# torgeiba/CPUPerformanceRayTracer

Measured on AMD Instinct MI355X. Metric: ray-samples/sec (pixels×spp×bounces) at 1920×1080; ms/frame, higher is better.
Workload: dtype f32; 1 GPU; c2_1080p; width=1920, height=1080, spp=8, bounces=8, parallelism=single GPU, step=one launch accumulating 8 frames (spp) of every pixel in HBM

## Files before the change

### cpuperformanceraytracer_amd/_native.py

```python
from __future__ import annotations

import ctypes
import os
from pathlib import Path

from .build import LIB as _LIB_PATH

PT_OK = 0
PT_EINVAL = -1
PT_EHIP = -2
PT_ENOMEM = -3
PT_ESTATE = -4
PT_EKERNEL = -5

PT_LAYOUT_INTERLEAVED = 0
PT_LAYOUT_PLANAR8 = 1
PT_LAYOUT_TILED_PLANAR8 = 2

PT_FLAG_DEFER_READBACK = 1
PT_FLAG_PIN_HOST = 2
PT_FLAG_GATHER_ROOT = 4

PT_MAX_DEVICES = 16

PT_PIXEL_RGBA8 = 0
PT_PIXEL_XRGB8 = 1

EXPORTED_SYMBOLS = (
    "pt_init", "pt_shutdown", "pt_last_error", "pt_default_config", "pt_set_frame", "pt_get_frame",
    "pt_render_scalar", "pt_render_simd", "pt_render_simd_tiled", "pt_render_tile", "pt_begin_frame",
    "pt_readback", "pt_gather_root", "pt_unpin_host", "pt_release_buffer", "pt_initialized_device", "pt_check_device_errors", "pt_build_checked", "pt_device_count",
    "pt_device_ordinal", "pt_render_device", "pt_render_device_chain", "pt_chain_counts", "pt_count_device", "pt_render_device_present", "pt_launch_variant",
    "pt_cam_cache_query",
    "pt_load_texture", "pt_decode_hdr", "pt_free_texture", "pt_set_env_map", "pt_render_simt_textured",
    "pt_tonemap", "pt_tonemap_device", "pt_write_bmp", "pt_load_cubemap_texture",
    "pt_v4_default_config", "pt_v4_set_config", "pt_v4_get_config", "pt_v4_initialize_global_render_resources",
    "pt_v4_reinitialize_render_tile_data", "pt_v4_initialize_scene", "pt_v4_clear_scene", "pt_v4_add_material",
    "pt_v4_add_quad", "pt_v4_add_sphere", "pt_v4_set_frame", "pt_v4_get_frame", "pt_v4_get_scene_tables", "pt_render_opt_v4",
    "pt_copy_output_to_file", "pt_v4_render_device", "pt_v4_render_device_chain", "pt_v4_count_device", "pt_v4_begin_frame",
    "pt_make_work_queue", "pt_add_work_queue_entry", "pt_complete_all_work", "pt_complete_all_work_async",
    "pt_wait_work", "pt_work_queue_size", "pt_free_work_queue",
)

PT_RENDERER_SIMD_TILED = 0
PT_RENDERER_SIMT_TEXTURED = 1
PT_RENDERER_V4 = 2

PT_V4_ENV_NONE = 0
PT_V4_ENV_EQUIRECT = 1
PT_V4_ENV_CUBEMAP = 2
PT_V4_MAX_OBJECTS = 12


class PtConfig(ctypes.Structure):
    _fields_ = [("device", ctypes.c_int32), ("num_bounces", ctypes.c_int32),
                ("samples_per_frame", ctypes.c_int32), ("flags", ctypes.c_uint32),
# ... 81 lines not shown
        "pt_set_frame": (i32, [u32]),
        "pt_get_frame": (u32, []),
        "pt_render_scalar": (i32, [vp, i32, i32, i32]),
        "pt_render_simd": (i32, [vp, i32, i32, i32]),
        "pt_render_simd_tiled": (i32, [vp, i32, i32, i32, i32, i32, i32, i32]),
        "pt_render_tile": (i32, [ctypes.POINTER(PtBufferInfo), ctypes.POINTER(PtTileInfo)]),
        "pt_begin_frame": (i32, []),
        "pt_readback": (i32, [vp]),
        "pt_gather_root": (i32, [vp, ctypes.POINTER(vp)]),
        "pt_unpin_host": (i32, [vp]),
        "pt_release_buffer": (i32, [vp]),
        "pt_initialized_device": (i32, []),
        "pt_check_device_errors": (i32, []),
        "pt_build_checked": (i32, []),
        "pt_device_count": (i32, []),
        "pt_device_ordinal": (i32, [i32]),
        "pt_render_device": (i32, [ctypes.POINTER(PtDeviceJob), vp]),
        "pt_count_device": (i32, [ctypes.POINTER(PtDeviceJob), vp, ctypes.POINTER(PtWorkCounts)]),
        "pt_render_device_present": (i32, [ctypes.POINTER(PtDeviceJob), vp, i32, vp]),
        "pt_render_device_chain": (i32, [ctypes.POINTER(PtDeviceJob), vp]),
        "pt_chain_counts": (i32, [ctypes.POINTER(ctypes.c_uint64), ctypes.POINTER(ctypes.c_uint64)]),
        "pt_launch_variant": (i32, [ctypes.POINTER(PtDeviceJob), ctypes.POINTER(i32), ctypes.POINTER(i32)]),
        "pt_cam_cache_query": (i32, [ctypes.POINTER(PtDeviceJob), vp, ctypes.POINTER(i32), ctypes.POINTER(ctypes.c_uint64)]),
        "pt_load_texture": (i32, [ctypes.c_char_p, ctypes.POINTER(PtTexture)]),
        "pt_decode_hdr": (i32, [vp, ctypes.c_size_t, ctypes.POINTER(PtTexture)]),
        "pt_free_texture": (None, [ctypes.POINTER(PtTexture)]),
        "pt_set_env_map": (i32, [ctypes.POINTER(PtTexture)]),
        "pt_render_simt_textured": (i32, [vp, i32, i32, i32, i32, i32, i32, i32, ctypes.POINTER(PtTexture)]),
        "pt_tonemap": (i32, [vp, i32, i32, i32, i32, i32, vp, i32]),
        "pt_tonemap_device": (i32, [vp, i32, i32, i32, i32, i32, vp, i32, vp]),
        "pt_write_bmp": (i32, [ctypes.c_char_p, i32, i32, i32, vp]),
        "pt_load_cubemap_texture": (i32, [ctypes.POINTER(ctypes.c_char_p), ctypes.POINTER(PtTexture)]),
        "pt_v4_default_config": (None, [ctypes.POINTER(PtV4Config)]),
        "pt_v4_set_config": (i32, [ctypes.POINTER(PtV4Config)]),
        "pt_v4_get_config": (i32, [ctypes.POINTER(PtV4Config)]),
        "pt_v4_initialize_global_render_resources": (i32, []),
        "pt_v4_reinitialize_render_tile_data": (i32, []),
        "pt_v4_initialize_scene": (i32, []),
        "pt_v4_clear_scene": (i32, []),
        "pt_v4_add_material": (i32, [ctypes.POINTER(PtV4Material)]),
        "pt_v4_add_quad": (i32, [ctypes.POINTER(ctypes.c_float)]),
        "pt_v4_add_sphere": (i32, [ctypes.POINTER(ctypes.c_float)]),
        "pt_v4_set_frame": (i32, [u32]),
        "pt_v4_get_frame": (u32, []),
        "pt_v4_get_scene_tables": (i32, [vp, i32, ctypes.POINTER(i32), ctypes.POINTER(i32)]),
        "pt_render_opt_v4": (i32, [vp, i32, i32, i32, i32, i32, i32, i32, ctypes.POINTER(PtTexture), vp]),
# ... 31 lines not shown
```

### cpuperformanceraytracer_amd/build.py

```python
from __future__ import annotations

import os
import shutil
import subprocess
import sys
from pathlib import Path

PKG = Path(__file__).resolve().parent
ROOT = PKG.parent
CSRC = PKG / "csrc"
LIB = PKG / "libpt_mi355.so"
ARCH = os.environ.get("PT_OFFLOAD_ARCH", "gfx950")

SOURCES = ["pt_kernel.hip", "pt_output.hip", "pt_v4.hip", "pt_scene.cpp", "pt_v4_scene.cpp", "pt_capi.cpp",
           "pt_dropin.cpp", "pt_texture.cpp"]
HEADERS = ["pt_kernel.h", "pt_output.h", "pt_v4.h", "pt_v4_default_scene.h", "pt_scene.h", "pt_sincosf.h", "pt_exactmath.h",
           "pt_invtrig.h", "pt_envcert.h", "pt_tile_queue.h", "pt_quadcull.h", "pt_libmf.h", "pt_wave.h", "pt_guard.h",
           "pt_chain.h", "pt_camcache.h"]
CHECKED_LIB = ROOT / "build" / "libpt_checked.so"
PARITY_FLAGS = [
    "-ffp-contract=off",
    "-fhip-fp32-correctly-rounded-divide-sqrt",
    "-fno-gpu-flush-denormals-to-zero",
]
PERF_FLAGS = ["-mllvm", "-amdgpu-atomic-optimizer-strategy=None", "-fno-slp-vectorize"]


def hipcc() -> str:
    for cand in (os.environ.get("HIPCC"), "/opt/rocm/bin/hipcc", shutil.which("hipcc")):
        if cand and Path(cand).exists():
            return cand
    raise RuntimeError("hipcc not found (ROCm required to build libpt_mi355.so)")


def _stale(target: Path, deps) -> bool:
    if not target.exists():
        return True
    t = target.stat().st_mtime
    return any(Path(d).stat().st_mtime > t for d in deps)


# ... 89 lines not shown
```

### cpuperformanceraytracer_amd/csrc/pt_capi.cpp

```cpp
#include "pt_kernel.h"
#include "pt_guard.h"
#include "pt_output.h"
#include "pt_v4.h"
#include "../../include/pt_mi355.h"
#include <stdarg.h>
#include <stdio.h>
#include <stdlib.h>
#include <string.h>
#include <new>
#include <vector>

namespace {

struct SchedKey {
    int32_t kind = 0;
    int32_t width = 0, height = 0, col0 = 0, ncols = 0, row_start = 0, row_stride = 0, nrows = 0, bounces = 0;
    const float* env = nullptr;
    uint32_t ntiles = 0;
    uint32_t split = 0;
    bool operator==(const SchedKey& o) const
    {
        return kind == o.kind && width == o.width && height == o.height && col0 == o.col0 && ncols == o.ncols &&
               row_start == o.row_start && row_stride == o.row_stride && nrows == o.nrows && bounces == o.bounces &&
               env == o.env && ntiles == o.ntiles && split == o.split;
    }
};
struct Sched {
    bool used = false;
    hipStream_t stream = nullptr;
    SchedKey key;
    uint32_t* cost = nullptr;
    uint32_t* order = nullptr;
    uint32_t* units = nullptr;
    bool have_cost = false;
    bool built = false;
    unsigned long long launches = 0;
    unsigned long long last_use = 0;
    hipEvent_t tune_ev[2 * 18] = {};
    uint32_t tuned = 0;
    uint32_t narms = 0;
    int32_t tune_nframes = 0;
    int8_t wide = -1;
    uint32_t* epoch = nullptr;
    uint32_t chain_seq = 0;
    unsigned long long* cam = nullptr;
    bool cam_off = false;
    uint8_t cam_state = 0;
};
enum : uint8_t { kCamEmpty = 0, kCamFilled = 1, kCamSettled = 2 };
constexpr uint32_t kTuneRounds = 3;
constexpr int kSchedSlots = 16;
constexpr int kBands = 4;
constexpr uint32_t kSchedMinTiles = 512;
constexpr unsigned kQueueRing = 256;
constexpr unsigned long long kSchedRebuildDefault = 256;

struct Dev {
    int32_t ordinal = 0;
    hipStream_t stream = nullptr;
    PtScene* dscene = nullptr;
    float* dbuf = nullptr;
    size_t dbuf_cap = 0;
    unsigned long long* dcounters = nullptr;
    uint32_t* derr = nullptr;
    float* dct = nullptr;
    uint32_t dct_waves = 0;
    int ct_slot = -1;
    uint32_t* herr = nullptr;
    unsigned int* dqueue = nullptr;
    unsigned queue_next = 0;
    bool queue_pre_zeroed = false;
    hipStream_t last_stream = nullptr;
    hipStream_t queue_stream[kQueueRing] = {};
    hipEvent_t queue_event[kQueueRing] = {};
    int16_t queue_alias[kQueueRing];
    float* denv = nullptr;
    Sched sched[kSchedSlots];
    unsigned long long sched_clock = 0;
    unsigned long long cam_checked = 0;
    float* dtone_in = nullptr;
    size_t dtone_in_cap = 0;
    uint32_t* dtone_out = nullptr;
    size_t dtone_out_cap = 0;
    float* dgather = nullptr;
    size_t dgather_cap = 0;
    hipEvent_t ev_gather = nullptr;
    bool peer_root = false;
    struct Chain {
        hipStream_t st[2] = {};
        hipEvent_t done[2] = {};
        bool pending[2] = {};
        hipEvent_t ev_caller = nullptr;
        float* area1 = nullptr;
        unsigned int* qblk = nullptr;
        unsigned long long* started = nullptr;
        unsigned long long cum = 0;
        Sched* sched = nullptr;
        int area = 0;
        int par = 0;
        unsigned long long restarts = 0, continued = 0;
        bool off = false;
// ... 25 lines not shown
    hipStream_t s_in = nullptr, s_out = nullptr;
    hipEvent_t ev_in[kBands] = {}, ev_done[kBands] = {};
    hipEvent_t ev_q = nullptr;
    hipEvent_t ev_root_free = nullptr;
    pt_v4_config v4cfg{PT_V4_ENV_EQUIRECT, 1, 1, 8, 1, 1, 1, 1, 1};
    bool v4_scene_ready = false;
    PtV4SceneDesc v4desc{};
    PtV4Scene v4scene{};
    uint32_t v4_frame = 0;
    uint32_t ring_guard_cap = ~0u;
    int32_t v4_ct_force = 0;
    uint32_t ct_back_pct = 20;
    bool back_set = false;
    uint32_t ct_waves = 0;
    char ct_seq[64] = {};
    uint32_t ct_seq_len = 0, ct_seq_pos = 0;
    uint32_t split = 1;
    int64_t test_bad_entry = -1;
    bool cam_cache = true;
    bool no_ct = false;
    uint32_t test_chain_delay = 0;
    uint32_t unit_mult = 2;
    unsigned long long sched_rebuild = kSchedRebuildDefault;
};

State g;
char g_err[512] = "no error";

int vfail(int code, const char* fmt, va_list ap)
{
    vsnprintf(g_err, sizeof(g_err), fmt, ap);
    return code;
}

int fail(int code, const char* fmt, ...)
{
    va_list ap;
    va_start(ap, fmt);
    vfail(code, fmt, ap);
    va_end(ap);
    return code;
}

#define HIP_TRY(expr)                                                                          \
    do {                                                                                       \
        hipError_t e_ = (expr);                                                                \
// ... 274 lines not shown
    j.order = nullptr;
    j.units = nullptr;
    j.nunits = nullptr;
    j.cost = nullptr;
    j.err = nullptr;
    j.guard_cap = g.ring_guard_cap;
    j.ct_slots = nullptr;
    j.ct_waves = 0;
    j.ct_back_pct = 0;
    j.ct_wide = 0;
    j.scene = nullptr;
    j.tile_epoch = nullptr;
    j.chain_seq = 0;
    j.chain_wait = 0;
    j.started = nullptr;
    j.cam_cache = nullptr;
    j.cam_mode = PT_CAM_NONE;
    return j;
}

void free_sched(Sched& s)
{
    if (s.cost) (void)hipFree(s.cost);
    if (s.order) (void)hipFree(s.order);
    if (s.units) (void)hipFree(s.units);
    if (s.epoch) (void)hipFree(s.epoch);
    if (s.cam) (void)hipFree(s.cam);
    for (hipEvent_t e : s.tune_ev)
        if (e) (void)hipEventDestroy(e);
    s = Sched{};
}

SchedKey sched_key(const PtJob& j)
{
    SchedKey k;
    k.kind = 0;
    k.width = j.width;
    k.height = j.height;
    k.col0 = j.col0;
    k.ncols = j.ncols;
    k.row_start = j.row_start;
    k.row_stride = j.row_stride;
    k.nrows = j.nrows;
    k.bounces = j.num_bounces;
    k.env = j.env;
    k.ntiles = pt_job_tiles(j);
    return k;
}
// ... 31 lines not shown
{
    j.cam_cache = nullptr;
    j.cam_mode = PT_CAM_NONE;
    if (!s || !j.ct_slots || !cam_launch_qualifies(*s, j.nframes)) return;
    if (s->cam_state == kCamFilled) s->cam_state = kCamSettled;
    if (s->cam_state == kCamEmpty && count) return;
    if (!s->cam) {
        const size_t bytes = pt_cam_cache_bytes(s->key.ntiles);
        if (hipMalloc(&s->cam, bytes) != hipSuccess || hipMemsetAsync(s->cam, 0xff, bytes, st) != hipSuccess) {
            (void)hipGetLastError();
            if (s->cam) (void)hipFree(s->cam);
            s->cam = nullptr;
            s->cam_off = true;
            return;
        }
    }
    j.cam_cache = s->cam;
    j.cam_mode = s->cam_state == kCamEmpty ? PT_CAM_FILL : PT_CAM_USE;
}

Sched* find_sched(Dev& dv, const SchedKey& key, hipStream_t st)
{
    const uint32_t n = key.ntiles;
    if (n < kSchedMinTiles) return nullptr;
    Sched* lru = &dv.sched[0];
    for (Sched& s : dv.sched) {
        if (s.used && s.stream == st && s.key == key) {
            s.last_use = ++dv.sched_clock;
            return &s;
        }
        if (!s.used || (lru->used && s.last_use < lru->last_use)) lru = &s;
    }
    if (lru->used) {
        (void)hipDeviceSynchronize();
        if (dv.chain.sched == lru) dv.chain.sched = nullptr;
        free_sched(*lru);
    }
    Sched s;
    if (hipMalloc(&s.cost, 2 * (size_t)n * sizeof(uint32_t)) != hipSuccess ||
        hipMalloc(&s.order, 2 * (size_t)n * sizeof(uint32_t)) != hipSuccess ||
        hipMalloc(&s.units, (2 * (size_t)n + 2) * sizeof(uint32_t)) != hipSuccess) {
        free_sched(s);
        return nullptr;
    }
    s.used = true;
    s.stream = st;
    s.key = key;
    s.last_use = ++dv.sched_clock;
    *lru = s;
    return lru;
}

int slot_event(Dev& dv, unsigned slot)
{
    if (!dv.queue_event[slot]) HIP_TRY(hipEventCreateWithFlags(&dv.queue_event[slot], hipEventDisableTiming));
    return PT_OK;
}

hipEvent_t slot_order(const Dev& dv, unsigned slot)
{
    const int a = dv.queue_alias[slot];
    return a >= 0 ? dv.queue_event[a] : dv.queue_event[slot];
}

struct LaunchSched {
    unsigned slot = 0;
    unsigned int* queue = nullptr;
    unsigned int* queue_next = nullptr;
    const uint32_t* order = nullptr;
    const uint32_t* units = nullptr;
    const uint32_t* nunits = nullptr;
    uint32_t* cost = nullptr;
    Sched* sched = nullptr;
    Sched* geo = nullptr;
};
int chain_join(Dev& dv, hipStream_t st)
{
    for (int i = 0; i < 2; ++i) {
        if (!dv.chain.pending[i]) continue;
        if (hipEventQuery(dv.chain.done[i]) == hipSuccess) {
            dv.chain.pending[i] = false;
        } else {
            (void)hipGetLastError();
            HIP_TRY(hipStreamWaitEvent(st, dv.chain.done[i], 0));
        }
    }
    dv.chain.sched = nullptr;
    return PT_OK;
}

int use_sched(Dev& dv, const SchedKey& key, hipStream_t st, LaunchSched* ls, uint32_t split,
              const hipStream_t* sched_st = nullptr)
{
    *ls = LaunchSched{};
    int rc;
    if ((rc = chain_join(dv, st))) return rc;
    if (Sched* s = find_sched(dv, key, sched_st ? *sched_st : st)) {
        ls->geo = s;
        if (s->have_cost && (!s->built || s->launches % g.sched_rebuild == 0)) {
            const uint32_t unit_mult = key.kind == 0 && !g.no_ct ? g.unit_mult : 1u;
            hipError_t e = pt_launch_schedule(s->cost, s->order, s->units, s->units + 2 * s->key.ntiles + 1, s->key.ntiles,
                                              split, unit_mult, st, dv.derr);
            if (e != hipSuccess) return fail(PT_EHIP, "schedule launch failed: %s", hipGetErrorString(e));
            s->built = true;
            if (g.test_bad_entry >= 0 && (uint32_t)g.test_bad_entry < 2u * s->key.ntiles)
                HIP_TRY(hipMemsetAsync(s->order + g.test_bad_entry, 0xff, sizeof(uint32_t), st));
        }
        if (s->built) {
            ls->sched = s;
            ls->order = s->order;
            ls->units = s->units;
            ls->nunits = s->units + 2 * s->key.ntiles + 1;
        }
        if (!s->built || (s->launches + 1) % g.sched_rebuild == 0) {
            ls->cost = s->cost;
            s->have_cost = true;
        }
        ++s->launches;
    }
    unsigned slot = dv.queue_next++ % kQueueRing;
    bool pre = dv.queue_pre_zeroed;
    if (pre && dv.last_stream != st) {
        const unsigned prev = (slot + kQueueRing - 1) % kQueueRing;
        dv.queue_alias[slot] = (int16_t)prev;
        dv.queue_stream[slot] = dv.queue_stream[prev];
        slot = dv.queue_next++ % kQueueRing;
        pre = false;
    }
    ls->slot = slot;
    if (hipEvent_t ev = slot_order(dv, slot); ev && dv.queue_stream[slot] != st) HIP_TRY(hipStreamWaitEvent(st, ev, 0));
    ls->queue = dv.dqueue + (size_t)slot * PT_QUEUE_WORDS;
    if (!pre) HIP_TRY(hipMemsetAsync(ls->queue, 0, PT_QUEUE_WORDS * sizeof(unsigned), st));
    dv.queue_pre_zeroed = false;
    const unsigned next = (slot + 1) % kQueueRing;
    if (hipEvent_t ev = slot_order(dv, next); ev && dv.queue_stream[next] != st) HIP_TRY(hipStreamWaitEvent(st, ev, 0));
    ls->queue_next = dv.dqueue + (size_t)next * PT_QUEUE_WORDS;
    return PT_OK;
}

int queue_done(Dev& dv, unsigned slot, hipStream_t st, bool zeroed_next)
{
// ... 188 lines not shown
int chain_continue(Dev& dv, PtV4Job& j, Sched*, hipStream_t X, uint32_t* blocks)
{
    if (j.env_mode != PT_V4_ENV_NONE) j.env = dv.denv;
    j.ct_force = g.v4_ct_force;
    j.ct_back_pct = j.nframes <= 16 ? (g.back_set ? g.ct_back_pct : kChainBack) : 0u;
    hipError_t e = pt_launch_v4(j, g.v4scene, X, false, nullptr, blocks);
    if (e != hipSuccess) return fail(PT_EHIP, "v4 render launch failed: %s", hipGetErrorString(e));
    return PT_OK;
}

template <typename Job>
int launch_chain(Dev& dv, Job j, hipStream_t s)
{
    int rc;
    if ((rc = use_dev(dv))) return rc;
    if (dv.chain.off) return chain_restart(dv, j, s, nullptr, nullptr);
    const SchedKey key = chain_key(j);
    Sched* sc = g.no_ct || j.ncols <= 0 || j.nrows <= 0 || j.nframes <= 0 ? nullptr : find_sched(dv, key, s);
    if (!sc) return chain_restart(dv, j, s, nullptr, nullptr);
    ct_area_alloc(dv);
    if ((rc = chain_setup(dv, *sc))) return rc;
    Dev::Chain& c = dv.chain;
    if (!dv.dct || !c.area1) return chain_restart(dv, j, s, nullptr, nullptr);
    const bool builds = sc->have_cost && (!sc->built || sc->launches % g.sched_rebuild == 0);
    const bool records = !sc->built || (sc->launches + 1) % g.sched_rebuild == 0;
    const bool cont = c.sched == sc && sc->built && !builds && chain_variant_fixed(j, *sc) &&
                      cam_chain_may_continue(*sc, j.nframes);
    const uint32_t seq = sc->chain_seq + 1;
    const int par = cont ? c.par ^ 1 : 0;
    hipStream_t X = c.st[par];
    j.tile_epoch = sc->epoch;
    j.chain_seq = seq;
    j.started = c.started;
    j.chain_delay = g.test_chain_delay;
    uint32_t blocks = 0;
    if (!cont) {
        HIP_TRY(hipEventRecord(c.ev_caller, s));
        HIP_TRY(hipStreamWaitEvent(X, c.ev_caller, 0));
        if ((rc = chain_join(dv, X))) return rc;
        HIP_TRY(hipMemsetAsync(c.qblk, 0, 4 * PT_QUEUE_WORDS * sizeof(unsigned), X));
        j.chain_wait = 0;
        if ((rc = chain_restart(dv, j, X, &blocks, &s))) return rc;
        c.area = 0;
    } else {
        HIP_TRY(hipStreamWaitValue64(X, c.started, c.cum, hipStreamWaitValueGte, ~0ull));
        j.chain_wait = seq - 1;
        j.queue = c.qblk + (size_t)(seq % 4u) * PT_QUEUE_WORDS;
        j.queue_next = c.qblk + (size_t)((seq + 2u) % 4u) * PT_QUEUE_WORDS;
        j.order = sc->order;
        j.units = sc->units;
        j.nunits = sc->units + 2 * sc->key.ntiles + 1;
        j.cost = records ? sc->cost : nullptr;
        if (records) sc->have_cost = true;
        j.err = dv.derr;
        c.area ^= 1;
        j.ct_slots = c.area ? c.area1 : dv.dct;
        j.ct_waves = dv.dct_waves;
        ++sc->launches;
        if ((rc = chain_continue(dv, j, sc, X, &blocks))) return rc;
    }
    c.cum += blocks;
    sc->chain_seq = seq;
    ++(cont ? c.continued : c.restarts);
    HIP_TRY(hipEventRecord(c.done[par], X));
    c.pending[par] = true;
    HIP_TRY(hipStreamWaitEvent(s, c.done[par], 0));
    c.sched = blocks ? sc : nullptr;
    c.par = par;
    return PT_OK;
}

void unpin()
{
    if (g.pinned) {
        (void)hipDeviceSynchronize();
        (void)hipHostUnregister((void*)g.pinned);
    }
    g.pinned = nullptr;
    g.pinned_bytes = 0;
}

bool pin(const float* p, size_t bytes)
// ... 462 lines not shown
    }
    if (n == 0) return 0;
    c->device = c->devices[0];
    c->device_count = n;
    return n;
}

void free_dev(Dev& dv)
{
    if (use_dev(dv)) return;
    if (dv.stream) (void)hipStreamSynchronize(dv.stream);
    if (dv.dbuf) (void)hipFree(dv.dbuf);
    if (dv.dcounters) (void)hipFree(dv.dcounters);
    if (dv.derr) (void)hipFree(dv.derr);
    if (dv.dct) (void)hipFree(dv.dct);
    if (dv.herr) (void)hipHostFree(dv.herr);
    if (dv.dscene) (void)hipFree(dv.dscene);
    if (dv.dqueue) (void)hipFree(dv.dqueue);
    if (dv.denv) (void)hipFree(dv.denv);
    if (dv.dtone_in) (void)hipFree(dv.dtone_in);
    if (dv.dtone_out) (void)hipFree(dv.dtone_out);
    if (dv.dgather) (void)hipFree(dv.dgather);
    if (dv.ev_gather) (void)hipEventDestroy(dv.ev_gather);
    for (Sched& sc : dv.sched)
        if (sc.used) free_sched(sc);
    for (hipEvent_t& e : dv.queue_event)
        if (e) (void)hipEventDestroy(e);
    for (int i = 0; i < 2; ++i) {
        if (dv.chain.st[i]) (void)hipStreamSynchronize(dv.chain.st[i]), (void)hipStreamDestroy(dv.chain.st[i]);
        if (dv.chain.done[i]) (void)hipEventDestroy(dv.chain.done[i]);
    }
    if (dv.chain.ev_caller) (void)hipEventDestroy(dv.chain.ev_caller);
    if (dv.chain.area1) (void)hipFree(dv.chain.area1);
    if (dv.chain.qblk) (void)hipFree(dv.chain.qblk);
    if (dv.chain.started) (void)hipFree(dv.chain.started);
    if (dv.stream) (void)hipStreamDestroy(dv.stream);
    dv = Dev{};
}

int init_dev(Dev& dv, int32_t ordinal)
{
    dv = Dev{};
    dv.ordinal = ordinal;
    for (int16_t& a : dv.queue_alias) a = -1;
    HIP_TRY(hipSetDevice(ordinal));
    HIP_TRY(hipStreamCreateWithFlags(&dv.stream, hipStreamNonBlocking));
// ... 91 lines not shown
        int can = 0;
        if (hipDeviceCanAccessPeer(&can, dv.ordinal, g.dev[0].ordinal) != hipSuccess || !can) continue;
        HIP_TRY(hipSetDevice(dv.ordinal));
        const hipError_t e = hipDeviceEnablePeerAccess(g.dev[0].ordinal, 0);
        if (e == hipSuccess || e == hipErrorPeerAccessAlreadyEnabled) dv.peer_root = true;
        (void)hipGetLastError();
    }
    HIP_TRY(hipSetDevice(g.dev[0].ordinal));
    HIP_TRY(hipEventCreateWithFlags(&g.ev_root_free, hipEventDisableTiming));
    HIP_TRY(hipStreamCreateWithFlags(&g.s_in, hipStreamNonBlocking));
    HIP_TRY(hipStreamCreateWithFlags(&g.s_out, hipStreamNonBlocking));
    for (int k = 0; k < kBands; ++k) {
        HIP_TRY(hipEventCreateWithFlags(&g.ev_in[k], hipEventDisableTiming));
        HIP_TRY(hipEventCreateWithFlags(&g.ev_done[k], hipEventDisableTiming));
    }
    HIP_TRY(hipEventCreateWithFlags(&g.ev_q, hipEventDisableTiming));
    g.frame = 0;
    g.ring_guard_cap = ~0u;
    g.cam_cache = !(getenv("PT_MI355_CAM_CACHE") && !strcmp(getenv("PT_MI355_CAM_CACHE"), "0"));
    g.no_ct = getenv("PT_MI355_NO_CT") && !strcmp(getenv("PT_MI355_NO_CT"), "1");
    g.test_chain_delay = getenv("PT_MI355_TEST_CHAIN_DELAY") ? (uint32_t)strtoul(getenv("PT_MI355_TEST_CHAIN_DELAY"), nullptr, 10) : 0u;
    g.sched_rebuild = getenv("PT_MI355_SCHED_REBUILD") ? std::max<unsigned long long>(2ull, strtoull(getenv("PT_MI355_SCHED_REBUILD"), nullptr, 10))
                                                        : kSchedRebuildDefault;
    g.unit_mult = getenv("PT_MI355_UNIT_MULT") ? std::max<uint32_t>(1u, (uint32_t)strtoul(getenv("PT_MI355_UNIT_MULT"), nullptr, 10)) : 2u;
    g.v4_ct_force = getenv("PT_MI355_V4_CT") && !strcmp(getenv("PT_MI355_V4_CT"), "1");
    g.ct_back_pct = 20;
    g.back_set = false;
    if (const char* bk = getenv("PT_MI355_BACK")) g.ct_back_pct = (uint32_t)strtoul(bk, nullptr, 10), g.back_set = true;
    g.ct_waves = 0;
    if (const char* cw = getenv("PT_MI355_CT_WAVES")) g.ct_waves = (uint32_t)strtoul(cw, nullptr, 10);
    g.ct_seq_len = g.ct_seq_pos = 0;
    if (const char* sq = getenv("PT_MI355_CT_WAVES_SEQ")) {
        for (const char* c = sq; *c && g.ct_seq_len < sizeof(g.ct_seq); ++c)
            if (*c == '5' || *c == '6') g.ct_seq[g.ct_seq_len++] = *c;
    }
    g.test_bad_entry = -1;
    if (const char* be = getenv("PT_MI355_TEST_BAD_ENTRY")) g.test_bad_entry = (int64_t)strtoll(be, nullptr, 10);
    g.split = 1;
    if (const char* sp = getenv("PT_MI355_SPLIT")) g.split = (uint32_t)strtoul(sp, nullptr, 10);
    if (const char* cap = getenv("PT_MI355_RING_GUARD_CAP")) {
        const unsigned long v = strtoul(cap, nullptr, 10);
        if (v > 0 && v < 0xfffffffful) g.ring_guard_cap = (uint32_t)v;
    }
    g.inited = true;
    return PT_OK;
}
// ... 347 lines not shown
    return launch(*dv, j, (hipStream_t)stream, false);
}

int pt_launch_variant(const pt_device_job* dj, int32_t* waves, int32_t* back_pct)
{
    int rc;
    PtJob j;
    Dev* dv = nullptr;
    if (!waves || !back_pct) return fail(PT_EINVAL, "null output");
    *waves = 0;
    *back_pct = 0;
    if ((rc = ensure_init()) || (rc = device_job(dj, &j)) || (rc = dev_of(dj->buf, &dv))) return rc;
    if (dj->use_env) j.env = dv->denv;
    if (g.no_ct) return PT_OK;
    const bool back = j.nframes <= 16;
    const uint32_t dflt = back ? g.ct_back_pct : 0u;
    if (g.ct_waves) {
        *waves = j.env ? pt_ct_env_waves() : (int32_t)g.ct_waves;
        *back_pct = (int32_t)dflt;
        return PT_OK;
    }
    SchedKey key = sched_key(j);
    key.split = j.nframes <= 8 ? g.split : 0u;
    if (key.ntiles < kSchedMinTiles) {
        *waves = j.env ? pt_ct_env_waves() : 5;
        *back_pct = (int32_t)dflt;
        return PT_OK;
    }
    for (const Sched& s : dv->sched) {
        if (!s.used || !(s.key == key) || s.wide < 0) continue;
        if (j.env) {
            *waves = pt_ct_env_waves();
            *back_pct = (int32_t)(s.wide && back && !g.back_set ? kEnvBack[s.wide] : dflt);
        } else {
            *waves = s.wide ? 6 : 5;
            *back_pct = (int32_t)(s.wide == 2 && back ? kBackWide : dflt);
        }
        return PT_OK;
    }
    return PT_OK;
}

int pt_count_device(const pt_device_job* dj, void* stream, pt_work_counts* out)
{
    int rc;
    PtJob j;
    Dev* dv = nullptr;
// ... 26 lines not shown
    out->sky_skipped = h[PT_CNT_SKY];
    dv->cam_checked = h[PT_CNT_CAM_CHECKED];
    return PT_OK;
}

int pt_cam_cache_query(const pt_device_job* dj, void* stream, int32_t* state, uint64_t* compared)
{
    int rc;
    PtJob j;
    Dev* dv = nullptr;
    if (!state || !compared) return fail(PT_EINVAL, "null output");
    *state = PT_CAM_CACHE_NONE;
    *compared = 0;
    if ((rc = ensure_init()) || (rc = device_job(dj, &j)) || (rc = dev_of(dj->buf, &dv))) return rc;
    if (dj->use_env) j.env = dv->denv;
    *compared = dv->cam_checked;
    SchedKey key = sched_key(j);
    key.split = j.nframes <= 8 ? g.split : 0u;
    for (const Sched& s : dv->sched) {
        if (!s.used || s.stream != (hipStream_t)stream || !(s.key == key)) continue;
        if (s.cam && cam_launch_qualifies(s, j.nframes))
            *state = s.cam_state == kCamEmpty ? PT_CAM_CACHE_EMPTY : s.cam_state == kCamFilled ? PT_CAM_CACHE_FILLED : PT_CAM_CACHE_SETTLED;
        break;
    }
    return PT_OK;
}

int pt_check_device_errors(void)
{
    if (!g.inited) return PT_OK;
    DeviceGuard guard;
    return sync_all();
}

int32_t pt_initialized_device(void) { return g.inited ? g.dev[0].ordinal : -1; }

int32_t pt_build_checked(void) { return PT_CHECKED ? 1 : 0; }

int32_t pt_device_count(void) { return g.inited ? g.ndev : 0; }

int32_t pt_device_ordinal(int32_t i) { return g.inited && i >= 0 && i < g.ndev ? g.dev[i].ordinal : -1; }

int pt_unpin_host(const void* buf)
{
    if (!g.inited || !g.pinned) return PT_OK;
    if (buf && buf != (const void*)g.pinned) return PT_OK;
// ... 510 lines not shown
```

### cpuperformanceraytracer_amd/device.py

```python
from __future__ import annotations

import ctypes

from . import _native as N


def ensure_backend(device_index: int, num_bounces: int = 4) -> None:
    from . import renderer
    cur = renderer.initialized_devices()
    if device_index in cur:
        return
    if cur:
        raise N.PtError(N.PT_ESTATE, "ensure_backend",
                        f"libpt_mi355 is initialised on devices {cur}; a job on device {device_index} needs "
                        "renderer.init(devices=[...]) naming it, or its own process")
    import torch
    prev = torch.cuda.current_device()
    try:
        renderer.init(num_bounces=num_bounces, device=device_index)
    finally:
        torch.cuda.set_device(prev)


def set_env_map(env, device_index: int = 0, num_bounces: int = 4) -> None:
# ... 53 lines not shown
                   row_stride: int = 1, nrows: int | None = None, layout: int = N.PT_LAYOUT_INTERLEAVED,
                   use_env: bool = False) -> dict:
    nrows = height if nrows is None else nrows
    job = _job(buf, width, height, row_start, row_stride, nrows, 1, nframes, num_bounces, layout, use_env)
    w, b = ctypes.c_int32(0), ctypes.c_int32(0)
    N.check(N.load().pt_launch_variant(ctypes.byref(job), ctypes.byref(w), ctypes.byref(b)), "pt_launch_variant")
    return {"waves_per_simd": int(w.value), "back_claim_pct": int(b.value)}


CAM_CACHE_STATES = ("none", "empty", "filled", "settled")


def cam_cache_query(buf, width: int, height: int, *, nframes: int, num_bounces: int, row_start: int = 0,
                    row_stride: int = 1, nrows: int | None = None, layout: int = N.PT_LAYOUT_INTERLEAVED,
                    use_env: bool = False, stream=None) -> dict:
    nrows = height if nrows is None else nrows
    job = _job(buf, width, height, row_start, row_stride, nrows, 1, nframes, num_bounces, layout, use_env)
    s, c = ctypes.c_int32(0), ctypes.c_uint64(0)
    N.check(N.load().pt_cam_cache_query(ctypes.byref(job), _stream(stream), ctypes.byref(s), ctypes.byref(c)),
            "pt_cam_cache_query")
    return {"state": CAM_CACHE_STATES[int(s.value)], "compared": int(c.value)}


def tonemap_device(buf, width: int, nrows: int, pixels, *, layout: int = N.PT_LAYOUT_INTERLEAVED,
                   pixel_format: int = N.PT_PIXEL_RGBA8, stream=None) -> None:
    _check_pixels(pixels, width * nrows, buf)
    N.check(N.load().pt_tonemap_device(buf.data_ptr(), width, nrows, layout, 0, 0, pixels.data_ptr(), pixel_format,
                                       _stream(stream)), "pt_tonemap_device")


def _check_pixels(pixels, n: int, buf) -> None:
    import torch
    if not isinstance(pixels, torch.Tensor) or pixels.device != buf.device:
        raise N.PtError(N.PT_EINVAL, "render_device_present", "pixels must be a tensor on the buffer's device")
    if pixels.element_size() != 4 or not pixels.is_contiguous() or pixels.numel() < n:
        raise N.PtError(N.PT_EINVAL, "render_device_present", f"pixels must hold >= {n} contiguous 32-bit words")


def count_device(buf, width: int, height: int, *, frame_first: int, nframes: int, num_bounces: int,
                 row_start: int = 0, row_stride: int = 1, nrows: int | None = None,
                 layout: int = N.PT_LAYOUT_INTERLEAVED, use_env: bool = False, stream=None) -> dict:
    nrows = height if nrows is None else nrows
    job = _job(buf, width, height, row_start, row_stride, nrows, frame_first, nframes, num_bounces, layout, use_env)
    out = N.PtWorkCounts()
    N.check(N.load().pt_count_device(ctypes.byref(job), _stream(stream), ctypes.byref(out)), "pt_count_device")
    return {"segments": out.segments, "lane_slots": out.lane_slots, "samples": out.samples, "escaped": out.escaped,
# ... 59 lines not shown
```

### include/pt_mi355.h

```cpp
#ifndef PT_MI355_H
#define PT_MI355_H
#include <stddef.h>
#include <stdint.h>
#ifdef __cplusplus
extern "C" {
#endif

#define PT_OK 0
#define PT_EINVAL (-1)
#define PT_EHIP (-2)
#define PT_ENOMEM (-3)
#define PT_ESTATE (-4)
#define PT_EKERNEL (-5)

#define PT_LAYOUT_INTERLEAVED 0
#define PT_LAYOUT_PLANAR8 1
#define PT_LAYOUT_TILED_PLANAR8 2

#define PT_FLAG_DEFER_READBACK 1u
#define PT_FLAG_PIN_HOST 2u
#define PT_FLAG_GATHER_ROOT 4u

#define PT_MAX_DEVICES 16

// ... 138 lines not shown
#define PT_RENDERER_V4 2
typedef struct pt_work_queue pt_work_queue;
pt_work_queue* pt_make_work_queue(int32_t renderer);
int pt_add_work_queue_entry(pt_work_queue* q, const pt_buffer_info* buffer, const pt_tile_info* tile);
int pt_complete_all_work(pt_work_queue* q);
int pt_complete_all_work_async(pt_work_queue* q);
int pt_wait_work(pt_work_queue* q);
int32_t pt_work_queue_size(const pt_work_queue* q);
void pt_free_work_queue(pt_work_queue* q);

int pt_render_device(const pt_device_job* job, void* hip_stream);
int pt_render_device_chain(const pt_device_job* job, void* hip_stream);
int pt_chain_counts(uint64_t* restarts, uint64_t* continued);
int pt_count_device(const pt_device_job* job, void* hip_stream, pt_work_counts* out);
int pt_render_device_present(const pt_device_job* job, uint32_t* pixels, int32_t format, void* hip_stream);
int pt_launch_variant(const pt_device_job* job, int32_t* waves, int32_t* back_pct);
enum {
    PT_CAM_CACHE_NONE = 0,
    PT_CAM_CACHE_EMPTY = 1,
    PT_CAM_CACHE_FILLED = 2,
    PT_CAM_CACHE_SETTLED = 3,
};
int pt_cam_cache_query(const pt_device_job* job, void* hip_stream, int32_t* state, uint64_t* compared);

#ifdef __cplusplus
}
#endif
#endif
```

Before: 624.3 billion ray-samples/s.

## Double-buffer tile schedule and rebuild it asynchronously on a side stream

Periodic tile-schedule rebuilds now write into an idle second order/units buffer on a separate non-blocking stream. The render keeps using the live buffer and swaps only once an event shows the build has finished. This takes the rebuild kernel off the render stream's critical path and lets the chained launch continue instead of restarting on rebuild frames. In exchange, launches may use a slightly stale schedule, memory for schedules doubles, and the swap logic and stream ordering become more complex.

```diff
diff --git a/cpuperformanceraytracer_amd/_native.py b/cpuperformanceraytracer_amd/_native.py
--- a/cpuperformanceraytracer_amd/_native.py
+++ b/cpuperformanceraytracer_amd/_native.py
@@ -31,7 +31,7 @@
     "pt_render_scalar", "pt_render_simd", "pt_render_simd_tiled", "pt_render_tile", "pt_begin_frame",
     "pt_readback", "pt_gather_root", "pt_unpin_host", "pt_release_buffer", "pt_initialized_device", "pt_check_device_errors", "pt_build_checked", "pt_device_count",
     "pt_device_ordinal", "pt_render_device", "pt_render_device_chain", "pt_chain_counts", "pt_count_device", "pt_render_device_present", "pt_launch_variant",
-    "pt_cam_cache_query",
+    "pt_cam_cache_query", "pt_sched_query",
     "pt_load_texture", "pt_decode_hdr", "pt_free_texture", "pt_set_env_map", "pt_render_simt_textured",
     "pt_tonemap", "pt_tonemap_device", "pt_write_bmp", "pt_load_cubemap_texture",
     "pt_v4_default_config", "pt_v4_set_config", "pt_v4_get_config", "pt_v4_initialize_global_render_resources",
@@ -159,6 +159,8 @@
         "pt_chain_counts": (i32, [ctypes.POINTER(ctypes.c_uint64), ctypes.POINTER(ctypes.c_uint64)]),
         "pt_launch_variant": (i32, [ctypes.POINTER(PtDeviceJob), ctypes.POINTER(i32), ctypes.POINTER(i32)]),
         "pt_cam_cache_query": (i32, [ctypes.POINTER(PtDeviceJob), vp, ctypes.POINTER(i32), ctypes.POINTER(ctypes.c_uint64)]),
+        "pt_sched_query": (i32, [ctypes.POINTER(PtDeviceJob), ctypes.POINTER(ctypes.c_uint64), ctypes.POINTER(ctypes.c_uint64),
+                                 ctypes.POINTER(i32)]),
         "pt_load_texture": (i32, [ctypes.c_char_p, ctypes.POINTER(PtTexture)]),
         "pt_decode_hdr": (i32, [vp, ctypes.c_size_t, ctypes.POINTER(PtTexture)]),
         "pt_free_texture": (None, [ctypes.POINTER(PtTexture)]),
diff --git a/cpuperformanceraytracer_amd/build.py b/cpuperformanceraytracer_amd/build.py
--- a/cpuperformanceraytracer_amd/build.py
+++ b/cpuperformanceraytracer_amd/build.py
@@ -16,7 +16,7 @@
            "pt_dropin.cpp", "pt_texture.cpp"]
 HEADERS = ["pt_kernel.h", "pt_output.h", "pt_v4.h", "pt_v4_default_scene.h", "pt_scene.h", "pt_sincosf.h", "pt_exactmath.h",
            "pt_invtrig.h", "pt_envcert.h", "pt_tile_queue.h", "pt_quadcull.h", "pt_libmf.h", "pt_wave.h", "pt_guard.h",
-           "pt_chain.h", "pt_camcache.h"]
+           "pt_chain.h", "pt_camcache.h", "pt_schedswap.h"]
 CHECKED_LIB = ROOT / "build" / "libpt_checked.so"
 PARITY_FLAGS = [
     "-ffp-contract=off",
diff --git a/cpuperformanceraytracer_amd/csrc/pt_capi.cpp b/cpuperformanceraytracer_amd/csrc/pt_capi.cpp
--- a/cpuperformanceraytracer_amd/csrc/pt_capi.cpp
+++ b/cpuperformanceraytracer_amd/csrc/pt_capi.cpp
@@ -2,6 +2,7 @@
 #include "pt_guard.h"
 #include "pt_output.h"
 #include "pt_v4.h"
+#include "pt_schedswap.h"
 #include "../../include/pt_mi355.h"
 #include <stdarg.h>
 #include <stdio.h>
@@ -30,11 +31,13 @@
     hipStream_t stream = nullptr;
     SchedKey key;
     uint32_t* cost = nullptr;
-    uint32_t* order = nullptr;
-    uint32_t* units = nullptr;
-    bool have_cost = false;
-    bool built = false;
-    unsigned long long launches = 0;
+    struct Set {
+        uint32_t* order = nullptr;
+        uint32_t* units = nullptr;
+    } set[2];
+    uint32_t* nunits(int i) const { return set[i].units + 2 * (size_t)key.ntiles + 1; }
+    PtSchedSwap sw;
+    hipEvent_t built_ev = nullptr;
     unsigned long long last_use = 0;
     hipEvent_t tune_ev[2 * 18] = {};
     uint32_t tuned = 0;
@@ -77,6 +80,8 @@
     float* denv = nullptr;
     Sched sched[kSchedSlots];
     unsigned long long sched_clock = 0;
+    hipStream_t sched_st = nullptr;
+    hipEvent_t sched_ev = nullptr;
     unsigned long long cam_checked = 0;
     float* dtone_in = nullptr;
     size_t dtone_in_cap = 0;
@@ -148,6 +153,7 @@
     uint32_t test_chain_delay = 0;
     uint32_t unit_mult = 2;
     unsigned long long sched_rebuild = kSchedRebuildDefault;
+    uint32_t sched_min_tiles = kSchedMinTiles;
 };
 
 State g;
@@ -468,8 +474,11 @@
 void free_sched(Sched& s)
 {
     if (s.cost) (void)hipFree(s.cost);
-    if (s.order) (void)hipFree(s.order);
-    if (s.units) (void)hipFree(s.units);
+    for (Sched::Set& t : s.set) {
+        if (t.order) (void)hipFree(t.order);
+        if (t.units) (void)hipFree(t.units);
+    }
+    if (s.built_ev) (void)hipEventDestroy(s.built_ev);
     if (s.epoch) (void)hipFree(s.epoch);
     if (s.cam) (void)hipFree(s.cam);
     for (hipEvent_t e : s.tune_ev)
@@ -547,7 +556,7 @@
 Sched* find_sched(Dev& dv, const SchedKey& key, hipStream_t st)
 {
     const uint32_t n = key.ntiles;
-    if (n < kSchedMinTiles) return nullptr;
+    if (n < g.sched_min_tiles) return nullptr;
     Sched* lru = &dv.sched[0];
     for (Sched& s : dv.sched) {
         if (s.used && s.stream == st && s.key == key) {
@@ -563,8 +572,10 @@
     }
     Sched s;
     if (hipMalloc(&s.cost, 2 * (size_t)n * sizeof(uint32_t)) != hipSuccess ||
-        hipMalloc(&s.order, 2 * (size_t)n * sizeof(uint32_t)) != hipSuccess ||
-        hipMalloc(&s.units, (2 * (size_t)n + 2) * sizeof(uint32_t)) != hipSuccess) {
+        hipMalloc(&s.set[0].order, 2 * (size_t)n * sizeof(uint32_t)) != hipSuccess ||
+        hipMalloc(&s.set[0].units, (2 * (size_t)n + 2) * sizeof(uint32_t)) != hipSuccess ||
+        hipMalloc(&s.set[1].order, 2 * (size_t)n * sizeof(uint32_t)) != hipSuccess ||
+        hipMalloc(&s.set[1].units, (2 * (size_t)n + 2) * sizeof(uint32_t)) != hipSuccess) {
         free_sched(s);
         return nullptr;
     }
@@ -599,7 +610,7 @@
     Sched* sched = nullptr;
     Sched* geo = nullptr;
 };
-int chain_join(Dev& dv, hipStream_t st)
+int chain_order(Dev& dv, hipStream_t st)
 {
     for (int i = 0; i < 2; ++i) {
         if (!dv.chain.pending[i]) continue;
@@ -610,7 +621,53 @@
             HIP_TRY(hipStreamWaitEvent(st, dv.chain.done[i], 0));
         }
     }
+    return PT_OK;
+}
+int chain_join(Dev& dv, hipStream_t st)
+{
+    int rc;
+    if ((rc = chain_order(dv, st))) return rc;
     dv.chain.sched = nullptr;
+    return PT_OK;
+}
+
+int sched_step(Dev& dv, Sched& s, hipStream_t st, bool chained, uint32_t split, PtSchedSwap* next, LaunchSched* ls)
+{
+    bool done = false;
+    if (s.sw.in_flight && !(done = hipEventQuery(s.built_ev) == hipSuccess)) (void)hipGetLastError();
+    *next = s.sw;
+    const PtSchedStep step = pt_schedswap_step(*next, g.sched_rebuild, done);
+    if (step.first_build || step.start_build) {
+        hipStream_t bst = st;
+        if (step.start_build) {
+            int rc;
+            if (!dv.sched_st) HIP_TRY(hipStreamCreateWithFlags(&dv.sched_st, hipStreamNonBlocking));
+            if (!s.built_ev) HIP_TRY(hipEventCreateWithFlags(&s.built_ev, hipEventDisableTiming));
+            bst = dv.sched_st;
+            if (chained) {
+                if ((rc = chain_order(dv, bst))) return rc;
+            } else {
+                if (!dv.sched_ev) HIP_TRY(hipEventCreateWithFlags(&dv.sched_ev, hipEventDisableTiming));
+                HIP_TRY(hipEventRecord(dv.sched_ev, st));
+                HIP_TRY(hipStreamWaitEvent(bst, dv.sched_ev, 0));
+            }
+        }
+        const uint32_t unit_mult = s.key.kind == 0 && !g.no_ct ? g.unit_mult : 1u;
+        const Sched::Set& t = s.set[step.target];
+        hipError_t e = pt_launch_schedule(s.cost, t.order, t.units, s.nunits(step.target), s.key.ntiles,
+                                          split, unit_mult, bst, dv.derr);
+        if (e != hipSuccess) return fail(PT_EHIP, "schedule launch failed: %s", hipGetErrorString(e));
+        if (g.test_bad_entry >= 0 && (uint32_t)g.test_bad_entry < 2u * s.key.ntiles)
+            HIP_TRY(hipMemsetAsync(t.order + g.test_bad_entry, 0xff, sizeof(uint32_t), bst));
+        if (step.start_build) HIP_TRY(hipEventRecord(s.built_ev, bst));
+    }
+    if (next->built) {
+        ls->sched = &s;
+        ls->order = s.set[step.live].order;
+        ls->units = s.set[step.live].units;
+        ls->nunits = s.nunits(step.live);
+    }
+    ls->cost = step.record ? s.cost : nullptr;
     return PT_OK;
 }
 
@@ -622,26 +679,9 @@
     if ((rc = chain_join(dv, st))) return rc;
     if (Sched* s = find_sched(dv, key, sched_st ? *sched_st : st)) {
         ls->geo = s;
-        if (s->have_cost && (!s->built || s->launches % g.sched_rebuild == 0)) {
-            const uint32_t unit_mult = key.kind == 0 && !g.no_ct ? g.unit_mult : 1u;
-            hipError_t e = pt_launch_schedule(s->cost, s->order, s->units, s->units + 2 * s->key.ntiles + 1, s->key.ntiles,
-                                              split, unit_mult, st, dv.derr);
-            if (e != hipSuccess) return fail(PT_EHIP, "schedule launch failed: %s", hipGetErrorString(e));
-            s->built = true;
-            if (g.test_bad_entry >= 0 && (uint32_t)g.test_bad_entry < 2u * s->key.ntiles)
-                HIP_TRY(hipMemsetAsync(s->order + g.test_bad_entry, 0xff, sizeof(uint32_t), st));
-        }
-        if (s->built) {
-            ls->sched = s;
-            ls->order = s->order;
-            ls->units = s->units;
-            ls->nunits = s->units + 2 * s->key.ntiles + 1;
-        }
-        if (!s->built || (s->launches + 1) % g.sched_rebuild == 0) {
-            ls->cost = s->cost;
-            s->have_cost = true;
-        }
-        ++s->launches;
+        PtSchedSwap next;
+        if ((rc = sched_step(dv, *s, st, false, split, &next, ls))) return rc;
+        s->sw = next;
     }
     unsigned slot = dv.queue_next++ % kQueueRing;
     bool pre = dv.queue_pre_zeroed;
@@ -876,9 +916,7 @@
     if ((rc = chain_setup(dv, *sc))) return rc;
     Dev::Chain& c = dv.chain;
     if (!dv.dct || !c.area1) return chain_restart(dv, j, s, nullptr, nullptr);
-    const bool builds = sc->have_cost && (!sc->built || sc->launches % g.sched_rebuild == 0);
-    const bool records = !sc->built || (sc->launches + 1) % g.sched_rebuild == 0;
-    const bool cont = c.sched == sc && sc->built && !builds && chain_variant_fixed(j, *sc) &&
+    const bool cont = c.sched == sc && sc->sw.built && chain_variant_fixed(j, *sc) &&
                       cam_chain_may_continue(*sc, j.nframes);
     const uint32_t seq = sc->chain_seq + 1;
     const int par = cont ? c.par ^ 1 : 0;
@@ -901,17 +939,20 @@
         j.chain_wait = seq - 1;
         j.queue = c.qblk + (size_t)(seq % 4u) * PT_QUEUE_WORDS;
         j.queue_next = c.qblk + (size_t)((seq + 2u) % 4u) * PT_QUEUE_WORDS;
-        j.order = sc->order;
-        j.units = sc->units;
-        j.nunits = sc->units + 2 * sc->key.ntiles + 1;
-        j.cost = records ? sc->cost : nullptr;
-        if (records) sc->have_cost = true;
+        PtSchedSwap next;
+        LaunchSched ls;
+        if ((rc = sched_step(dv, *sc, X, true, key.split, &next, &ls))) return rc;
+        j.order = ls.order;
+        j.units = ls.units;
+        j.nunits = ls.nunits;
+        j.cost = ls.cost;
         j.err = dv.derr;
-        c.area ^= 1;
-        j.ct_slots = c.area ? c.area1 : dv.dct;
+        const int area = c.area ^ 1;
+        j.ct_slots = area ? c.area1 : dv.dct;
         j.ct_waves = dv.dct_waves;
-        ++sc->launches;
         if ((rc = chain_continue(dv, j, sc, X, &blocks))) return rc;
+        c.area = area;
+        sc->sw = next;
     }
     c.cum += blocks;
     sc->chain_seq = seq;
@@ -1420,6 +1461,8 @@
     if (dv.dtone_out) (void)hipFree(dv.dtone_out);
     if (dv.dgather) (void)hipFree(dv.dgather);
     if (dv.ev_gather) (void)hipEventDestroy(dv.ev_gather);
+    if (dv.sched_st) (void)hipStreamSynchronize(dv.sched_st), (void)hipStreamDestroy(dv.sched_st);
+    if (dv.sched_ev) (void)hipEventDestroy(dv.sched_ev);
     for (Sched& sc : dv.sched)
         if (sc.used) free_sched(sc);
     for (hipEvent_t& e : dv.queue_event)
@@ -1557,6 +1600,8 @@
     g.test_chain_delay = getenv("PT_MI355_TEST_CHAIN_DELAY") ? (uint32_t)strtoul(getenv("PT_MI355_TEST_CHAIN_DELAY"), nullptr, 10) : 0u;
     g.sched_rebuild = getenv("PT_MI355_SCHED_REBUILD") ? std::max<unsigned long long>(2ull, strtoull(getenv("PT_MI355_SCHED_REBUILD"), nullptr, 10))
                                                         : kSchedRebuildDefault;
+    g.sched_min_tiles = kSchedMinTiles;
+    if (const char* mt = getenv("PT_MI355_TEST_SCHED_MIN_TILES")) g.sched_min_tiles = std::max<uint32_t>(1u, (uint32_t)strtoul(mt, nullptr, 10));
     g.unit_mult = getenv("PT_MI355_UNIT_MULT") ? std::max<uint32_t>(1u, (uint32_t)strtoul(getenv("PT_MI355_UNIT_MULT"), nullptr, 10)) : 2u;
     g.v4_ct_force = getenv("PT_MI355_V4_CT") && !strcmp(getenv("PT_MI355_V4_CT"), "1");
     g.ct_back_pct = 20;
@@ -1950,7 +1995,7 @@
     }
     SchedKey key = sched_key(j);
     key.split = j.nframes <= 8 ? g.split : 0u;
-    if (key.ntiles < kSchedMinTiles) {
+    if (key.ntiles < g.sched_min_tiles) {
         *waves = j.env ? pt_ct_env_waves() : 5;
         *back_pct = (int32_t)dflt;
         return PT_OK;
@@ -2023,6 +2068,28 @@
         if (s.cam && cam_launch_qualifies(s, j.nframes))
             *state = s.cam_state == kCamEmpty ? PT_CAM_CACHE_EMPTY : s.cam_state == kCamFilled ? PT_CAM_CACHE_FILLED : PT_CAM_CACHE_SETTLED;
         break;
+    }
+    return PT_OK;
+}
+
+int pt_sched_query(const pt_device_job* dj, uint64_t* builds_started, uint64_t* swaps, int32_t* build_in_flight)
+{
+    int rc;
+    PtJob j;
+    Dev* dv = nullptr;
+    if (!builds_started || !swaps || !build_in_flight) return fail(PT_EINVAL, "null output");
+    *builds_started = *swaps = 0;
+    *build_in_flight = 0;
+    if ((rc = ensure_init()) || (rc = device_job(dj, &j)) || (rc = dev_of(dj->buf, &dv))) return rc;
+    const SchedKey key = sched_key(j);
+    for (const Sched& s : dv->sched) {
+        const SchedKey& k = s.key;
+        if (!s.used || k.width != key.width || k.height != key.height || k.col0 != key.col0 || k.ncols != key.ncols ||
+            k.row_start != key.row_start || k.row_stride != key.row_stride || k.nrows != key.nrows || k.bounces != key.bounces)
+            continue;
+        *builds_started += s.sw.builds_started;
+        *swaps += s.sw.swaps;
+        *build_in_flight += s.sw.in_flight ? 1 : 0;
     }
     return PT_OK;
 }
diff --git a/cpuperformanceraytracer_amd/csrc/pt_schedswap.h b/cpuperformanceraytracer_amd/csrc/pt_schedswap.h
--- /dev/null
+++ b/cpuperformanceraytracer_amd/csrc/pt_schedswap.h
@@ -0,0 +1,70 @@
+#pragma once
+#include <stdint.h>
+
+struct PtSchedSwap {
+    uint64_t launches = 0;
+    bool have_cost = false;
+    bool built = false;
+    bool cost_fresh = false;
+    bool in_flight = false;
+    uint8_t live = 0;
+    int64_t idle_reader = -1;
+    uint64_t builds_started = 0;
+    uint64_t swaps = 0;
+    uint64_t skipped = 0;
+};
+
+struct PtSchedStep {
+    bool swap = false;
+    bool first_build = false;
+    bool start_build = false;
+    bool record = false;
+    uint8_t live = 0;
+    uint8_t target = 0;
+};
+
+constexpr uint8_t pt_schedswap_idle(const PtSchedSwap& s) { return (uint8_t)(s.live ^ 1u); }
+
+constexpr bool pt_schedswap_due(uint64_t n, uint64_t period) { return period != 0 && n % period == 0; }
+constexpr bool pt_schedswap_records(uint64_t n, uint64_t period) { return pt_schedswap_due(n + 1, period); }
+
+constexpr bool pt_schedswap_may_swap(const PtSchedSwap& s, bool built_done) { return s.in_flight && built_done; }
+
+inline PtSchedStep pt_schedswap_step(PtSchedSwap& s, uint64_t period, bool built_done)
+{
+    PtSchedStep st;
+    const uint64_t n = s.launches;
+    if (pt_schedswap_may_swap(s, built_done)) {
+        s.live ^= 1u;
+        s.in_flight = false;
+        s.idle_reader = (int64_t)n - 1;
+        ++s.swaps;
+        st.swap = true;
+    }
+    if (s.have_cost && !s.built) {
+        st.first_build = true;
+        st.target = s.live;
+        s.built = true;
+    } else if (s.built && s.have_cost && pt_schedswap_due(n, period)) {
+        if (s.cost_fresh && !s.in_flight) {
+            st.start_build = true;
+            st.target = pt_schedswap_idle(s);
+            s.in_flight = true;
+            ++s.builds_started;
+        } else {
+            ++s.skipped;
+        }
+    }
+    s.cost_fresh = false;
+    if (!s.built) {
+        st.record = true;
+        s.have_cost = true;
+    } else if (pt_schedswap_records(n, period) && !s.in_flight) {
+        st.record = true;
+        s.have_cost = true;
+        s.cost_fresh = true;
+    }
+    st.live = s.live;
+    ++s.launches;
+    return st;
+}
diff --git a/cpuperformanceraytracer_amd/device.py b/cpuperformanceraytracer_amd/device.py
--- a/cpuperformanceraytracer_amd/device.py
+++ b/cpuperformanceraytracer_amd/device.py
@@ -99,6 +99,16 @@
     return {"state": CAM_CACHE_STATES[int(s.value)], "compared": int(c.value)}
 
 
+def sched_query(buf, width: int, height: int, *, num_bounces: int, row_start: int = 0, row_stride: int = 1,
+                nrows: int | None = None) -> dict:
+    nrows = height if nrows is None else nrows
+    job = _job(buf, width, height, row_start, row_stride, nrows, 1, 1, num_bounces, N.PT_LAYOUT_INTERLEAVED)
+    b, s, f = ctypes.c_uint64(0), ctypes.c_uint64(0), ctypes.c_int32(0)
+    N.check(N.load().pt_sched_query(ctypes.byref(job), ctypes.byref(b), ctypes.byref(s), ctypes.byref(f)),
+            "pt_sched_query")
+    return {"builds_started": int(b.value), "swaps": int(s.value), "build_in_flight": int(f.value)}
+
+
 def tonemap_device(buf, width: int, nrows: int, pixels, *, layout: int = N.PT_LAYOUT_INTERLEAVED,
                    pixel_format: int = N.PT_PIXEL_RGBA8, stream=None) -> None:
     _check_pixels(pixels, width * nrows, buf)
diff --git a/include/pt_mi355.h b/include/pt_mi355.h
--- a/include/pt_mi355.h
+++ b/include/pt_mi355.h
@@ -184,6 +184,7 @@
     PT_CAM_CACHE_SETTLED = 3,
 };
 int pt_cam_cache_query(const pt_device_job* job, void* hip_stream, int32_t* state, uint64_t* compared);
+int pt_sched_query(const pt_device_job* job, uint64_t* builds_started, uint64_t* swaps, int32_t* build_in_flight);
 
 #ifdef __cplusplus
 }
```

Result: no change. 629.6 billion ray-samples/s (median of 6 runs) (+0.8%).
